# yahoojapan/srgd

Hardware: AMD Instinct MI355X
Metric: HR tiles/sec (256->1024 x4, 50 steps, CFG=1.0) (higher is better)
Workload: dtype bf16; 1 GPU; BASELINE configs[1]: one 256x256 LR tile x4 SR per step, 50 DDPM steps, class_cond_scale=1.0, dim-128 U-Net, bf16, device Philox noise; 5 steps (HR tiles) advance in lock-step so their U-Net tiles share launches; images_in_lockstep=5, step_lanes=1, tiles_per_unet_launch=125, parallelism=image-sharded x1

## Files before the change

### srgd_amd/csrc/conv1x1_bf16.hip

```cpp
#include "conv1x1_epilogue.hpp"

namespace srgd {
namespace {

constexpr int BM1 = 256, BN1 = 128, KC1 = 32, NT1 = 512;
constexpr int A1_BYTES = BM1 * KC1 * 2;
constexpr int B1_BYTES = BN1 * KC1 * 2;
constexpr int STAGE1 = A1_BYTES + B1_BYTES;
constexpr int RING1 = 3;
constexpr int LDS1_BYTES = RING1 * STAGE1;
static_assert(LDS1_BYTES >= EPI_LDS_BYTES && BM1 == EPI_BM && BN1 == EPI_BN && NT1 == EPI_NT, "conv1x1_epilogue.hpp tile shape");

typedef __attribute__((address_space(3))) void* lds_ptr1;
__device__ __forceinline__ void dma16_1(__amdgpu_buffer_rsrc_t rsrc, char* lds_wave_base, int voffset, int soffset) {
  __builtin_amdgcn_raw_ptr_buffer_load_lds(rsrc, (lds_ptr1)lds_wave_base, 16, voffset, soffset, 0, 0);
}
#define WAIT_VM1(N) asm volatile("s_waitcnt vmcnt(" #N ")" ::: "memory")
#define BARRIER1()                       \
  do {                                   \
    __builtin_amdgcn_s_barrier();        \
    __builtin_amdgcn_sched_barrier(0);   \
  } while (0)

struct Conv1Args {
  const bf16* in0; const bf16* in1; int C0, C1;
  int B, Hin, Win;
  int Hout, Wout;
  int KH, KW, stride;
  int ps0, ps1;
  const bf16* w;
  const float* bias;
  int Cout;
  bf16* out;
  const bf16* aux;
  const float* gn_a; const float* gn_b;
  unsigned char* oq; unsigned char* os;
  float* eps4; const float* fin_w; const float* fin_b;
};

__device__ __forceinline__ int row_swz1(int row) { return (row >> 1) & 3; }

template <int EPI>
__global__ __launch_bounds__(NT1, 4) void conv1x1_bf16_kernel(Conv1Args p) {
  extern __shared__ __attribute__((aligned(16))) char smem[];
  const int tid = threadIdx.x;
  const int lane = tid & 63;
  const int wave = __builtin_amdgcn_readfirstlane(tid >> 6);
  const int wm = wave >> 1, wn = wave & 1;
  const int r16 = lane & 15, q16 = lane >> 4;

  const int n_tiles = p.Cout / BN1;
  const int HWo = p.Hout * p.Wout;
  int wg = blockIdx.x;
  {
    const int nwg = gridDim.x, q = nwg >> 3, rem = nwg & 7, x = wg & 7, k = wg >> 3;
    wg = (x < rem ? x * (q + 1) : rem * (q + 1) + (x - rem) * q) + k;
  }
  const int nt = wg % n_tiles;
  const int mt = wg / n_tiles;
  const long m0 = (long)mt * BM1;
  const int b = (int)(m0 / HWo);
  const int p0 = (int)(m0 - (long)b * HWo);
  const int Cin = p.C0 + p.C1;
  const int CC = Cin / KC1;
  const int S = p.KH * p.KW * CC;

#define K_A1_DECL(J)                                                      \
  int a_b0##J, a_b1##J;                                                      \
  {                                                                          \
    const int g = (wave + 8 * J) * 64 + lane;                                \
    const int P = g >> 2;                                                    \
    const int op = p0 + P;                                                   \
    const int oy = op / p.Wout, ox = op - oy * p.Wout;                       \
    const int pix = oy * p.stride * p.Win + ox * p.stride;                   \
    const int sub = (g & 3) ^ row_swz1(P);                                   \
    a_b0##J = (pix * p.ps0 + sub * 8) * 2;                                   \
    a_b1##J = (pix * p.ps1 + sub * 8) * 2;                                   \
  }
  K_A1_DECL(0) K_A1_DECL(1)
#undef K_A1_DECL
  const size_t img0 = (size_t)p.Hin * p.Win * p.ps0, img1 = (size_t)p.Hin * p.Win * p.ps1;
  const __amdgpu_buffer_rsrc_t rs0 =
      __builtin_amdgcn_make_buffer_rsrc((void*)(p.in0 + (size_t)b * img0), 0, (int)(img0 * 2), 0x00020000);
  const __amdgpu_buffer_rsrc_t rs1 = __builtin_amdgcn_make_buffer_rsrc(
      (void*)(p.in1 ? p.in1 + (size_t)b * img1 : p.in0), 0, p.in1 ? (int)(img1 * 2) : 0, 0x00020000);
  const size_t w_tile_stride = (size_t)n_tiles * B1_BYTES;
  const __amdgpu_buffer_rsrc_t rsw = __builtin_amdgcn_make_buffer_rsrc(
      (void*)((const char*)p.w + (size_t)nt * B1_BYTES), 0, (int)((size_t)(S - 1) * w_tile_stride + B1_BYTES), 0x00020000);

  int i_ty = 0, i_tx = 0, i_cc = 0, i_slot = 0, i_w = 0;
  const int tid16 = tid * 16;
  auto issue = [&]() __attribute__((always_inline)) {
    const int c = i_cc * KC1;
    const bool first = c < p.C0;
    const int soff = first ? ((i_ty * p.Win + i_tx) * p.ps0 + c) * 2 : ((i_ty * p.Win + i_tx) * p.ps1 + c - p.C0) * 2;
    char* st = smem + i_slot * STAGE1;
    const int vo0 = first ? a_b00 : a_b10, vo1 = first ? a_b01 : a_b11;
    if (first) {
      dma16_1(rs0, st + wave * 1024, vo0, soff);
      dma16_1(rs0, st + (wave + 8) * 1024, vo1, soff);
    } else {
      dma16_1(rs1, st + wave * 1024, vo0, soff);
      dma16_1(rs1, st + (wave + 8) * 1024, vo1, soff);
    }
    dma16_1(rsw, st + A1_BYTES + wave * 1024, tid16, i_w);
    i_w += (int)w_tile_stride;
    i_slot = i_slot == RING1 - 1 ? 0 : i_slot + 1;
    if (++i_cc == CC) {
      i_cc = 0;
      if (++i_tx == p.KW) { i_tx = 0; ++i_ty; }
    }
  };

  f32x4 c00 = 0, c01 = 0, c02 = 0, c03 = 0, c10 = 0, c11 = 0, c12 = 0, c13 = 0,
        c20 = 0, c21 = 0, c22 = 0, c23 = 0, c30 = 0, c31 = 0, c32 = 0, c33 = 0;
  auto a_addr = [&](int i) {
    const int P = wm * 64 + i * 16 + r16;
    return P * 64 + ((q16 ^ row_swz1(P)) << 4);
  };
  auto b_addr = [&](int j) {
    const int n = wn * 64 + j * 16 + r16;
    return A1_BYTES + n * 64 + ((q16 ^ row_swz1(n)) << 4);
  };
  const int aa0 = a_addr(0), aa1 = a_addr(1), aa2 = a_addr(2), aa3 = a_addr(3);
  const int ba0 = b_addr(0), ba1 = b_addr(1), ba2 = b_addr(2), ba3 = b_addr(3);
  int c_slot = 0;
  auto compute = [&]() __attribute__((always_inline)) {
    const char* st = smem + c_slot * STAGE1;
    c_slot = c_slot == RING1 - 1 ? 0 : c_slot + 1;
    const bf16x8 a0 = *reinterpret_cast<const bf16x8*>(st + aa0);
    const bf16x8 a1 = *reinterpret_cast<const bf16x8*>(st + aa1);
    const bf16x8 a2 = *reinterpret_cast<const bf16x8*>(st + aa2);
    const bf16x8 a3 = *reinterpret_cast<const bf16x8*>(st + aa3);
    const bf16x8 b0 = *reinterpret_cast<const bf16x8*>(st + ba0);
    const bf16x8 b1 = *reinterpret_cast<const bf16x8*>(st + ba1);
    const bf16x8 b2 = *reinterpret_cast<const bf16x8*>(st + ba2);
    const bf16x8 b3 = *reinterpret_cast<const bf16x8*>(st + ba3);
#define MM(C_, A_, B_) C_ = __builtin_amdgcn_mfma_f32_16x16x32_bf16(A_, B_, C_, 0, 0, 0)
    MM(c00, a0, b0); MM(c01, a0, b1); MM(c02, a0, b2); MM(c03, a0, b3);
    MM(c10, a1, b0); MM(c11, a1, b1); MM(c12, a1, b2); MM(c13, a1, b3);
    MM(c20, a2, b0); MM(c21, a2, b1); MM(c22, a2, b2); MM(c23, a2, b3);
    MM(c30, a3, b0); MM(c31, a3, b1); MM(c32, a3, b2); MM(c33, a3, b3);
#undef MM
  };

  issue();
  if (S > 1) issue();
  if (S > 1) WAIT_VM1(3); else WAIT_VM1(0);
  BARRIER1();
  for (int s = 0; s < S; ++s) {
    if (s + 2 < S) issue();
    compute();
    if (s + 2 < S) WAIT_VM1(3); else WAIT_VM1(0);
    BARRIER1();
  }

  conv1x1_epilogue<EPI, BM1>(p, smem, tid, nt, m0, b, p0, c00, c01, c02, c03, c10, c11, c12, c13, c20, c21, c22, c23, c30, c31, c32, c33);
}

}

bool conv1x1_bf16_eligible(const ConvArgs& a) {
  if (a.pad != 0 || a.stride < 1 || a.KH < 1 || a.KW < 1) return false;
  if ((a.Hout - 1) * a.stride + a.KH > a.Hin || (a.Wout - 1) * a.stride + a.KW > a.Win) return false;
  if (a.ps0 % 8 || (a.C1 && (a.ps1 % 8 || a.ps1 < a.C1))) return false;
  if (a.ps0 != a.C0 && (a.C1 || (long)(a.Win - (a.Wout - 1) * a.stride - a.KW) * a.ps0 + a.ps0 < a.C0)) return false;
  if (a.C1 && (a.KH != 1 || a.KW != 1)) return false;
  if (a.C0 % KC1 || a.C1 % KC1 || a.Cout % BN1 || a.Cout != a.CoutPad) return false;
  if (((long)a.Hout * a.Wout) % BM1) return false;
  if (a.gn_partial) return false;
  if (a.mode == CONV_PIXEL_SHUFFLE_SILU && ((a.Cout / 4) % BN1 || a.residual || a.gn_res_src)) return false;
  if (a.mode != CONV_PLAIN && a.mode != CONV_PIXEL_SHUFFLE_SILU) return false;
  if (a.residual && a.gn_res_src) return false;
  if (a.eps4 && (!a.gn_res_src || a.Cout != BN1 || !a.fin_w || !a.fin_b || a.out_q)) return false;
  if ((size_t)a.Hin * a.Win * (size_t)std::max(a.ps0, a.ps1) * 2 >= (1ull << 31)) return false;
  if ((size_t)a.KH * a.KW * ((a.C0 + a.C1) / KC1) * (a.Cout / BN1) * B1_BYTES >= (1ull << 31)) return false;
  return true;
}

void pack_conv1x1_bf16(const float* src_tap_o_i, int taps, int Cin, int Cout, std::vector<unsigned short>& out,
                       unsigned short (*to_bf16)(float)) {
  const int CC = Cin / KC1, NTL = Cout / BN1;
  out.assign((size_t)taps * CC * NTL * BN1 * KC1, 0);
  for (int tap = 0; tap < taps; ++tap)
    for (int cc = 0; cc < CC; ++cc)
      for (int nt = 0; nt < NTL; ++nt) {
        unsigned short* tile = out.data() + ((size_t)(tap * CC + cc) * NTL + nt) * BN1 * KC1;
        for (int n = 0; n < BN1; ++n)
          for (int c = 0; c < 4; ++c) {
            const int cs = c ^ ((n >> 1) & 3);
            for (int e = 0; e < 8; ++e) {
              const int ci = cc * KC1 + c * 8 + e, o = nt * BN1 + n;
              tile[n * KC1 + cs * 8 + e] = to_bf16(src_tap_o_i[((size_t)tap * Cout + o) * Cin + ci]);
            }
          }
      }
}

int conv1x1_bf16(const ConvArgs& a, const void* packed_w, hipStream_t st) {
  if (!conv1x1_bf16_eligible(a)) SRGD_FAIL("conv1x1_bf16: shape not eligible");
  Conv1Args p;
  p.in0 = (const bf16*)a.in0; p.in1 = (const bf16*)a.in1; p.C0 = a.C0; p.C1 = a.C1;
  p.B = a.B; p.Hin = a.Hin; p.Win = a.Win; p.Hout = a.Hout; p.Wout = a.Wout;
  p.KH = a.KH; p.KW = a.KW; p.stride = a.stride; p.ps0 = a.ps0; p.ps1 = a.C1 ? a.ps1 : 0;
  p.w = (const bf16*)packed_w; p.bias = a.bias; p.Cout = a.Cout; p.out = (bf16*)a.out;
  p.aux = a.gn_res_src ? (const bf16*)a.gn_res_src : (const bf16*)a.residual;
  p.gn_a = a.gn_res_a; p.gn_b = a.gn_res_b;
  p.oq = (unsigned char*)a.out_q; p.os = (unsigned char*)a.out_s;
  p.eps4 = a.eps4; p.fin_w = a.fin_w; p.fin_b = a.fin_b;
  if ((p.oq != nullptr) != (p.os != nullptr)) SRGD_FAIL("conv1x1_bf16: MX-fp8 twin needs both the element and the scale buffer");
  const long m_tiles = (long)a.B * a.Hout * a.Wout / BM1;
  const long grid = m_tiles * (a.Cout / BN1);
  if (grid <= 0 || grid > 0x7fffffffL) SRGD_FAIL("conv1x1_bf16: bad grid");
  static bool attr_set[64] = {};
  if (DeviceSetup once(attr_set); once.need) {
#define K_SET1(E_)                                                                                   \
  SRGD_HIP(hipFuncSetAttribute(reinterpret_cast<const void*>(&conv1x1_bf16_kernel<E_>),                 \
                               hipFuncAttributeMaxDynamicSharedMemorySize, LDS1_BYTES));
    K_SET1(EPI_PLAIN) K_SET1(EPI_RESIDUAL) K_SET1(EPI_GNTAIL) K_SET1(EPI_PS_SILU) K_SET1(EPI_GNTAIL_FINAL)
#undef K_SET1
    once.done();
  }
#define K_GO1(E_) hipLaunchKernelGGL((conv1x1_bf16_kernel<E_>), dim3((unsigned)grid), dim3(NT1), LDS1_BYTES, st, p)
  if (a.mode == CONV_PIXEL_SHUFFLE_SILU) K_GO1(EPI_PS_SILU);
  else if (a.gn_res_src && a.eps4) K_GO1(EPI_GNTAIL_FINAL);
  else if (a.gn_res_src) K_GO1(EPI_GNTAIL);
  else if (a.residual) K_GO1(EPI_RESIDUAL);
  else K_GO1(EPI_PLAIN);
#undef K_GO1
  SRGD_HIP(hipGetLastError());
  return 0;
}

}
```

### srgd_amd/csrc/conv1x1_epilogue.hpp

```cpp
#pragma once
#include "kernels.hpp"

namespace srgd {
namespace {

enum { EPI_PLAIN = 0, EPI_RESIDUAL = 1, EPI_GNTAIL = 2, EPI_PS_SILU = 3, EPI_GNTAIL_FINAL = 4 };
constexpr int EPI_BM = 256, EPI_BN = 128, EPI_NT = 512;
constexpr int EPI_ROW = EPI_BN * 2 + 16;
constexpr int EPI_LDS_BYTES = EPI_BM * EPI_ROW;

template <int EPI, int BM, class Args>
__device__ __forceinline__ void conv1x1_epilogue(const Args& p, char* smem, const int tid, const int nt, const long m0, const int b,
                                                 const int p0, const f32x4& c00, const f32x4& c01, const f32x4& c02, const f32x4& c03,
                                                 const f32x4& c10, const f32x4& c11, const f32x4& c12, const f32x4& c13,
                                                 const f32x4& c20, const f32x4& c21, const f32x4& c22, const f32x4& c23,
                                                 const f32x4& c30, const f32x4& c31, const f32x4& c32, const f32x4& c33) {
  constexpr int BM1 = BM, BN1 = EPI_BN, NT1 = BM * 2, EROW1 = EPI_ROW;
  static_assert(BM == 256 || BM == 128, "conv1x1_epilogue: tile of 256 or 128 pixels");
  const int lane = tid & 63;
  const int wave = tid >> 6;
  const int wm = wave >> 1, wn = wave & 1;
  const int r16 = lane & 15, q16 = lane >> 4;
#pragma unroll
  for (int ni = 0; ni < 4; ++ni) {
    const int cl = wn * 64 + ni * 16 + r16;
    const float bias = p.bias ? p.bias[nt * BN1 + cl] : 0.f;
#pragma unroll
    for (int mi = 0; mi < 4; ++mi) {
      const f32x4 av = mi == 0 ? (ni == 0 ? c00 : ni == 1 ? c01 : ni == 2 ? c02 : c03)
                     : mi == 1 ? (ni == 0 ? c10 : ni == 1 ? c11 : ni == 2 ? c12 : c13)
                     : mi == 2 ? (ni == 0 ? c20 : ni == 1 ? c21 : ni == 2 ? c22 : c23)
                               : (ni == 0 ? c30 : ni == 1 ? c31 : ni == 2 ? c32 : c33);
      char* trow = smem + (wm * 64 + mi * 16 + q16 * 4) * EROW1 + cl * 2;
      float v0 = av[0] + bias, v1 = av[1] + bias, v2 = av[2] + bias, v3 = av[3] + bias;
      if (EPI == EPI_PS_SILU) { v0 = silu<false>(v0); v1 = silu<false>(v1); v2 = silu<false>(v2); v3 = silu<false>(v3); }
      typedef __bf16 bf16x2_t __attribute__((ext_vector_type(2)));
      const unsigned own01 = __builtin_bit_cast(unsigned, __builtin_convertvector(f32x2{v0, v1}, bf16x2_t));
      const unsigned own23 = __builtin_bit_cast(unsigned, __builtin_convertvector(f32x2{v2, v3}, bf16x2_t));
      const bool odd_lane = (r16 & 1) != 0;
      const unsigned recv = (unsigned)__builtin_amdgcn_update_dpp(0, (int)(odd_lane ? own01 : own23), 0xB1, 0xf, 0xf, true);
      const unsigned lo_ch = odd_lane ? recv : own01, hi_ch = odd_lane ? own23 : recv;
      char* prow = trow + (odd_lane ? 2 * EROW1 - 2 : 0);
      *reinterpret_cast<unsigned*>(prow) = __builtin_amdgcn_perm(hi_ch, lo_ch, 0x05040100u);
      *reinterpret_cast<unsigned*>(prow + EROW1) = __builtin_amdgcn_perm(hi_ch, lo_ch, 0x07060302u);
    }
  }
  __syncthreads();
  const int col0 = nt * BN1;
  size_t obase;
  int CoutPS = 0, ps_ij = 0, ps_c0 = 0;
  if (EPI == EPI_PS_SILU) {
    CoutPS = p.Cout >> 2;
    ps_ij = col0 / CoutPS;
    ps_c0 = col0 - ps_ij * CoutPS;
  }
  obase = (size_t)m0 * p.Cout + col0;
  float fw0[8], fw1[8], fw2[8];
  if (EPI == EPI_GNTAIL_FINAL) {
#pragma unroll
    for (int e = 0; e < 8; ++e) {
      fw0[e] = p.fin_w[(tid & 15) * 8 + e];
      fw1[e] = p.fin_w[BN1 + (tid & 15) * 8 + e];
      fw2[e] = p.fin_w[2 * BN1 + (tid & 15) * 8 + e];
    }
  }
  constexpr int NCH = (BM1 * 16) / NT1;
  bf16x8 auxv[NCH];
  f32x4 a_lo = {0.f, 0.f, 0.f, 0.f}, a_hi = a_lo, b_lo = a_lo, b_hi = a_lo;
  if (EPI == EPI_RESIDUAL || EPI == EPI_GNTAIL || EPI == EPI_GNTAIL_FINAL) {
#pragma unroll
    for (int i = 0; i < NCH; ++i) {
      const int q = tid + NT1 * i;
      const bf16x8* ap = reinterpret_cast<const bf16x8*>(p.aux + obase + (size_t)(q >> 4) * p.Cout + (q & 15) * 8);
      auxv[i] = __builtin_nontemporal_load(ap);
    }
    if (EPI != EPI_RESIDUAL) {
      const float* ga = p.gn_a + (size_t)b * p.Cout + col0 + (tid & 15) * 8;
      const float* gb = p.gn_b + (size_t)b * p.Cout + col0 + (tid & 15) * 8;
      a_lo = *reinterpret_cast<const f32x4*>(ga); a_hi = *reinterpret_cast<const f32x4*>(ga + 4);
      b_lo = *reinterpret_cast<const f32x4*>(gb); b_hi = *reinterpret_cast<const f32x4*>(gb + 4);
    }
  }
#pragma unroll
  for (int i = 0; i < NCH; ++i) {
    const int q = tid + NT1 * i;
    const int pix = q >> 4, c16 = q & 15;
    bf16x8 v = *reinterpret_cast<const bf16x8*>(smem + pix * EROW1 + c16 * 16);
    if (EPI == EPI_PS_SILU) {
      const int op = p0 + pix;
      const int oy = op / p.Wout, ox = op - oy * p.Wout;
      const size_t o = ((size_t)(b * 2 * p.Hout + 2 * oy + (ps_ij >> 1)) * (2 * p.Wout) + 2 * ox + (ps_ij & 1)) * CoutPS +
                       ps_c0 + c16 * 8;
      __builtin_nontemporal_store(v, reinterpret_cast<bf16x8*>(p.out + o));
      if (p.oq) mx_store_twin(v, p.oq, p.os, o, tid & 3);
    } else {
      const size_t o = obase + (size_t)pix * p.Cout + c16 * 8;
      if (EPI == EPI_RESIDUAL) {
        const bf16x8 rr = auxv[i];
#pragma unroll
        for (int e = 0; e < 8; ++e) v[e] = (bf16)((float)v[e] + (float)rr[e]);
      } else if (EPI == EPI_GNTAIL || EPI == EPI_GNTAIL_FINAL) {
        const bf16x8 hh = auxv[i];
#pragma unroll
        for (int e = 0; e < 8; ++e) {
          const float ca = e < 4 ? a_lo[e & 3] : a_hi[e & 3], cb = e < 4 ? b_lo[e & 3] : b_hi[e & 3];
          v[e] = (bf16)(silu<false>(ca * (float)hh[e] + cb) + (float)v[e]);
        }
      }
      if (EPI == EPI_GNTAIL_FINAL) {
        float s0 = 0.f, s1 = 0.f, s2 = 0.f;
#pragma unroll
        for (int e = 0; e < 8; ++e) {
          const float xv = (float)v[e];
          s0 += xv * fw0[e];
          s1 += xv * fw1[e];
          s2 += xv * fw2[e];
        }
        s0 = row16_sum(s0);
        s1 = row16_sum(s1);
        s2 = row16_sum(s2);
        if (c16 == 0)
          *reinterpret_cast<f32x4*>(p.eps4 + ((size_t)m0 + pix) * 4) = f32x4{s0 + p.fin_b[0], s1 + p.fin_b[1], s2 + p.fin_b[2], 0.f};
        continue;
      }
      __builtin_nontemporal_store(v, reinterpret_cast<bf16x8*>(p.out + o));
      if (p.oq) mx_store_twin(v, p.oq, p.os, o, tid & 3);
    }
  }
}

}
}
```

Before: 1.379 HR tiles/s.

## Make conv1x1 kernel persistent with cross-tile prefetch and round-based epilogue

The 1x1 conv GEMM kernel becomes persistent. The grid is capped at twice the CU count and each workgroup loops over output tiles. The next tile's DMA loads are issued while the current tile's last K-steps compute, which hides the pipeline fill and launch cost per tile. The epilogue is split into four rounds that stage 64 rows at a time through one ring slot instead of the whole LDS, and GN coefficients and final weights are cached in LDS. This adds loop and address bookkeeping plus more registers per thread, which risks occupancy and adds complexity.

Result: no change. 1.382 HR tiles/s, median of 4 (+0.2%).

```diff
diff --git a/srgd_amd/csrc/conv1x1_bf16.hip b/srgd_amd/csrc/conv1x1_bf16.hip
--- a/srgd_amd/csrc/conv1x1_bf16.hip
+++ b/srgd_amd/csrc/conv1x1_bf16.hip
@@ -9,7 +9,7 @@
 constexpr int STAGE1 = A1_BYTES + B1_BYTES;
 constexpr int RING1 = 3;
 constexpr int LDS1_BYTES = RING1 * STAGE1;
-static_assert(LDS1_BYTES >= EPI_LDS_BYTES && BM1 == EPI_BM && BN1 == EPI_BN && NT1 == EPI_NT, "conv1x1_epilogue.hpp tile shape");
+static_assert(STAGE1 >= EPI_RND_LDS && BM1 == EPI_BM && BN1 == EPI_BN && NT1 == EPI_NT, "conv1x1_epilogue.hpp tile shape");
 
 typedef __attribute__((address_space(3))) void* lds_ptr1;
 __device__ __forceinline__ void dma16_1(__amdgpu_buffer_rsrc_t rsrc, char* lds_wave_base, int voffset, int soffset) {
@@ -36,6 +36,7 @@
   const float* gn_a; const float* gn_b;
   unsigned char* oq; unsigned char* os;
   float* eps4; const float* fin_w; const float* fin_b;
+  int n_wg_tiles;
 };
 
 __device__ __forceinline__ int row_swz1(int row) { return (row >> 1) & 3; }
@@ -49,53 +50,61 @@
   const int wm = wave >> 1, wn = wave & 1;
   const int r16 = lane & 15, q16 = lane >> 4;
 
-  const int n_tiles = p.Cout / BN1;
-  const int HWo = p.Hout * p.Wout;
-  int wg = blockIdx.x;
-  {
-    const int nwg = gridDim.x, q = nwg >> 3, rem = nwg & 7, x = wg & 7, k = wg >> 3;
-    wg = (x < rem ? x * (q + 1) : rem * (q + 1) + (x - rem) * q) + k;
-  }
-  const int nt = wg % n_tiles;
-  const int mt = wg / n_tiles;
-  const long m0 = (long)mt * BM1;
-  const int b = (int)(m0 / HWo);
-  const int p0 = (int)(m0 - (long)b * HWo);
+  const unsigned n_tiles = p.Cout / BN1;
+  const unsigned tpi = (unsigned)(p.Hout * p.Wout) / BM1;
   const int Cin = p.C0 + p.C1;
   const int CC = Cin / KC1;
   const int S = p.KH * p.KW * CC;
-
-#define K_A1_DECL(J)                                                      \
-  int a_b0##J, a_b1##J;                                                      \
+  const int T = p.n_wg_tiles;
+  auto tile_of = [&](int v, int& nt_, int& mt_, int& b_, int& p0_) __attribute__((always_inline)) {
+    const int q = T >> 3, rem = T & 7, x = v & 7, k = v >> 3;
+    const unsigned wg = (x < rem ? x * (q + 1) : rem * (q + 1) + (x - rem) * q) + k;
+    nt_ = (int)(wg % n_tiles);
+    mt_ = (int)(wg / n_tiles);
+    b_ = (int)((unsigned)mt_ / tpi);
+    p0_ = (mt_ - b_ * (int)tpi) * BM1;
+  };
+
+  const int a_sub16 = ((lane & 3) ^ ((lane >> 3) & 3)) * 16;
+  int a_px0, a_px1, n_px0 = 0, n_px1 = 0;
+  auto lane_offsets = [&](const int v, int& px0, int& px1) __attribute__((always_inline)) {
+    int nt_, mt_, b_, p0_;
+    tile_of(v < T ? v : 0, nt_, mt_, b_, p0_);
+#define K_A1_SET(J)                                                       \
   {                                                                          \
-    const int g = (wave + 8 * J) * 64 + lane;                                \
-    const int P = g >> 2;                                                    \
-    const int op = p0 + P;                                                   \
+    const int op = p0_ + (((wave + 8 * J) * 64 + lane) >> 2);                \
     const int oy = op / p.Wout, ox = op - oy * p.Wout;                       \
-    const int pix = oy * p.stride * p.Win + ox * p.stride;                   \
-    const int sub = (g & 3) ^ row_swz1(P);                                   \
-    a_b0##J = (pix * p.ps0 + sub * 8) * 2;                                   \
-    a_b1##J = (pix * p.ps1 + sub * 8) * 2;                                   \
-  }
-  K_A1_DECL(0) K_A1_DECL(1)
-#undef K_A1_DECL
-  const size_t img0 = (size_t)p.Hin * p.Win * p.ps0, img1 = (size_t)p.Hin * p.Win * p.ps1;
-  const __amdgpu_buffer_rsrc_t rs0 =
-      __builtin_amdgcn_make_buffer_rsrc((void*)(p.in0 + (size_t)b * img0), 0, (int)(img0 * 2), 0x00020000);
-  const __amdgpu_buffer_rsrc_t rs1 = __builtin_amdgcn_make_buffer_rsrc(
-      (void*)(p.in1 ? p.in1 + (size_t)b * img1 : p.in0), 0, p.in1 ? (int)(img1 * 2) : 0, 0x00020000);
-  const size_t w_tile_stride = (size_t)n_tiles * B1_BYTES;
-  const __amdgpu_buffer_rsrc_t rsw = __builtin_amdgcn_make_buffer_rsrc(
-      (void*)((const char*)p.w + (size_t)nt * B1_BYTES), 0, (int)((size_t)(S - 1) * w_tile_stride + B1_BYTES), 0x00020000);
-
-  int i_ty = 0, i_tx = 0, i_cc = 0, i_slot = 0, i_w = 0;
-  const int tid16 = tid * 16;
-  auto issue = [&]() __attribute__((always_inline)) {
+    px##J = (oy * p.stride * p.Win + ox * p.stride) * 2;                     \
+  }
+    K_A1_SET(0) K_A1_SET(1)
+#undef K_A1_SET
+  };
+  lane_offsets(blockIdx.x, a_px0, a_px1);
+  const int img0 = p.Hin * p.Win * p.ps0, img1 = p.Hin * p.Win * p.ps1;
+  const int w_tile_stride = (int)n_tiles * B1_BYTES;
+
+  int i_v = blockIdx.x, i_ty = 0, i_tx = 0, i_cc = 0, i_slot = 0, i_w = 0;
+  __amdgpu_buffer_rsrc_t rs0, rs1, rsw;
+  auto issue_tile = [&]() __attribute__((always_inline)) {
+    int nt_, mt_, b_, p0_;
+    tile_of(i_v < T ? i_v : 0, nt_, mt_, b_, p0_);
+    rs0 = __builtin_amdgcn_make_buffer_rsrc((void*)(p.in0 + (size_t)b_ * img0), 0, img0 * 2, 0x00020000);
+    rs1 = __builtin_amdgcn_make_buffer_rsrc((void*)(p.in1 ? p.in1 + (size_t)b_ * img1 : p.in0), 0, p.in1 ? img1 * 2 : 0, 0x00020000);
+    rsw = __builtin_amdgcn_make_buffer_rsrc((void*)((const char*)p.w + (size_t)nt_ * B1_BYTES), 0,
+                                            (S - 1) * w_tile_stride + B1_BYTES, 0x00020000);
+    i_ty = i_tx = i_cc = 0;
+    i_w = 0;
+  };
+  issue_tile();
+  const int lane16 = lane * 16;
+  auto issue = [&]() __attribute__((always_inline)) -> bool {
+    if (i_v >= T) return false;
     const int c = i_cc * KC1;
     const bool first = c < p.C0;
     const int soff = first ? ((i_ty * p.Win + i_tx) * p.ps0 + c) * 2 : ((i_ty * p.Win + i_tx) * p.ps1 + c - p.C0) * 2;
     char* st = smem + i_slot * STAGE1;
-    const int vo0 = first ? a_b00 : a_b10, vo1 = first ? a_b01 : a_b11;
+    const int ps = first ? p.ps0 : p.ps1;
+    const int vo0 = a_px0 * ps + a_sub16, vo1 = a_px1 * ps + a_sub16;
     if (first) {
       dma16_1(rs0, st + wave * 1024, vo0, soff);
       dma16_1(rs0, st + (wave + 8) * 1024, vo1, soff);
@@ -103,39 +112,38 @@
       dma16_1(rs1, st + wave * 1024, vo0, soff);
       dma16_1(rs1, st + (wave + 8) * 1024, vo1, soff);
     }
-    dma16_1(rsw, st + A1_BYTES + wave * 1024, tid16, i_w);
-    i_w += (int)w_tile_stride;
+    dma16_1(rsw, st + A1_BYTES + wave * 1024, lane16, i_w + wave * 1024);
+    i_w += w_tile_stride;
     i_slot = i_slot == RING1 - 1 ? 0 : i_slot + 1;
     if (++i_cc == CC) {
       i_cc = 0;
-      if (++i_tx == p.KW) { i_tx = 0; ++i_ty; }
+      if (++i_tx == p.KW) {
+        i_tx = 0;
+        if (++i_ty == p.KH) {
+          i_v += gridDim.x;
+          a_px0 = n_px0; a_px1 = n_px1;
+          issue_tile();
+        }
+      }
     }
-  };
-
-  f32x4 c00 = 0, c01 = 0, c02 = 0, c03 = 0, c10 = 0, c11 = 0, c12 = 0, c13 = 0,
-        c20 = 0, c21 = 0, c22 = 0, c23 = 0, c30 = 0, c31 = 0, c32 = 0, c33 = 0;
-  auto a_addr = [&](int i) {
-    const int P = wm * 64 + i * 16 + r16;
-    return P * 64 + ((q16 ^ row_swz1(P)) << 4);
-  };
-  auto b_addr = [&](int j) {
-    const int n = wn * 64 + j * 16 + r16;
-    return A1_BYTES + n * 64 + ((q16 ^ row_swz1(n)) << 4);
-  };
-  const int aa0 = a_addr(0), aa1 = a_addr(1), aa2 = a_addr(2), aa3 = a_addr(3);
-  const int ba0 = b_addr(0), ba1 = b_addr(1), ba2 = b_addr(2), ba3 = b_addr(3);
+    return true;
+  };
+
+  f32x4 c00, c01, c02, c03, c10, c11, c12, c13, c20, c21, c22, c23, c30, c31, c32, c33;
+  const int aa0 = (wm * 64 + r16) * 64 + ((q16 ^ row_swz1(r16)) << 4);
+  const int ba0 = A1_BYTES + (wn * 64 + r16) * 64 + ((q16 ^ row_swz1(r16)) << 4);
   int c_slot = 0;
   auto compute = [&]() __attribute__((always_inline)) {
     const char* st = smem + c_slot * STAGE1;
     c_slot = c_slot == RING1 - 1 ? 0 : c_slot + 1;
     const bf16x8 a0 = *reinterpret_cast<const bf16x8*>(st + aa0);
-    const bf16x8 a1 = *reinterpret_cast<const bf16x8*>(st + aa1);
-    const bf16x8 a2 = *reinterpret_cast<const bf16x8*>(st + aa2);
-    const bf16x8 a3 = *reinterpret_cast<const bf16x8*>(st + aa3);
+    const bf16x8 a1 = *reinterpret_cast<const bf16x8*>(st + aa0 + 1024);
+    const bf16x8 a2 = *reinterpret_cast<const bf16x8*>(st + aa0 + 2048);
+    const bf16x8 a3 = *reinterpret_cast<const bf16x8*>(st + aa0 + 3072);
     const bf16x8 b0 = *reinterpret_cast<const bf16x8*>(st + ba0);
-    const bf16x8 b1 = *reinterpret_cast<const bf16x8*>(st + ba1);
-    const bf16x8 b2 = *reinterpret_cast<const bf16x8*>(st + ba2);
-    const bf16x8 b3 = *reinterpret_cast<const bf16x8*>(st + ba3);
+    const bf16x8 b1 = *reinterpret_cast<const bf16x8*>(st + ba0 + 1024);
+    const bf16x8 b2 = *reinterpret_cast<const bf16x8*>(st + ba0 + 2048);
+    const bf16x8 b3 = *reinterpret_cast<const bf16x8*>(st + ba0 + 3072);
 #define MM(C_, A_, B_) C_ = __builtin_amdgcn_mfma_f32_16x16x32_bf16(A_, B_, C_, 0, 0, 0)
     MM(c00, a0, b0); MM(c01, a0, b1); MM(c02, a0, b2); MM(c03, a0, b3);
     MM(c10, a1, b0); MM(c11, a1, b1); MM(c12, a1, b2); MM(c13, a1, b3);
@@ -144,18 +152,31 @@
 #undef MM
   };
 
-  issue();
-  if (S > 1) issue();
-  if (S > 1) WAIT_VM1(3); else WAIT_VM1(0);
+  bool more = issue();
+  more = issue() && more;
+  if (more) WAIT_VM1(3); else WAIT_VM1(0);
   BARRIER1();
-  for (int s = 0; s < S; ++s) {
-    if (s + 2 < S) issue();
-    compute();
-    if (s + 2 < S) WAIT_VM1(3); else WAIT_VM1(0);
-    BARRIER1();
-  }
-
-  conv1x1_epilogue<EPI, BM1>(p, smem, tid, nt, m0, b, p0, c00, c01, c02, c03, c10, c11, c12, c13, c20, c21, c22, c23, c30, c31, c32, c33);
+  for (int v = blockIdx.x; v < T; v += gridDim.x) {
+    int nt, mt, b, p0;
+    tile_of(v, nt, mt, b, p0);
+    lane_offsets(v + (int)gridDim.x, n_px0, n_px1);
+    c00 = 0; c01 = 0; c02 = 0; c03 = 0; c10 = 0; c11 = 0; c12 = 0; c13 = 0;
+    c20 = 0; c21 = 0; c22 = 0; c23 = 0; c30 = 0; c31 = 0; c32 = 0; c33 = 0;
+    for (int s = 0; s < S; ++s) {
+      const bool issued = issue();
+      compute();
+      if (s == 0 && v != (int)blockIdx.x) { if (issued) WAIT_VM1(11); else WAIT_VM1(8); }
+      else if (issued) WAIT_VM1(3);
+      else WAIT_VM1(0);
+      BARRIER1();
+    }
+    char* stg = smem + (c_slot == 0 ? RING1 - 1 : c_slot - 1) * STAGE1;
+    int tid_e = tid;
+    asm volatile("" : "+v"(tid_e));
+    conv1x1_epilogue_rounds<EPI>(p, stg, tid_e, nt, (long)mt * BM1, b, p0, c00, c01, c02, c03, c10, c11, c12, c13, c20, c21, c22, c23,
+                                 c30, c31, c32, c33);
+    EPI_LDS_BARRIER();
+  }
 }
 
 }
@@ -167,6 +188,7 @@
   if (a.ps0 != a.C0 && (a.C1 || (long)(a.Win - (a.Wout - 1) * a.stride - a.KW) * a.ps0 + a.ps0 < a.C0)) return false;
   if (a.C1 && (a.KH != 1 || a.KW != 1)) return false;
   if (a.C0 % KC1 || a.C1 % KC1 || a.Cout % BN1 || a.Cout != a.CoutPad) return false;
+  if (a.KH * a.KW * ((a.C0 + a.C1) / KC1) < 2) return false;
   if (((long)a.Hout * a.Wout) % BM1) return false;
   if (a.gn_partial) return false;
   if (a.mode == CONV_PIXEL_SHUFFLE_SILU && ((a.Cout / 4) % BN1 || a.residual || a.gn_res_src)) return false;
@@ -210,8 +232,19 @@
   p.eps4 = a.eps4; p.fin_w = a.fin_w; p.fin_b = a.fin_b;
   if ((p.oq != nullptr) != (p.os != nullptr)) SRGD_FAIL("conv1x1_bf16: MX-fp8 twin needs both the element and the scale buffer");
   const long m_tiles = (long)a.B * a.Hout * a.Wout / BM1;
-  const long grid = m_tiles * (a.Cout / BN1);
-  if (grid <= 0 || grid > 0x7fffffffL) SRGD_FAIL("conv1x1_bf16: bad grid");
+  const long tiles = m_tiles * (a.Cout / BN1);
+  if (tiles <= 0 || tiles > 0x7fff0000L) SRGD_FAIL("conv1x1_bf16: bad grid");
+  p.n_wg_tiles = (int)tiles;
+  static int cus[64] = {};
+  int dev = 0;
+  SRGD_HIP(hipGetDevice(&dev));
+  if (dev >= 0 && dev < 64 && cus[dev] == 0) {
+    int n = 0;
+    SRGD_HIP(hipDeviceGetAttribute(&n, hipDeviceAttributeMultiprocessorCount, dev));
+    __atomic_store_n(&cus[dev], n > 8 ? n & ~7 : 8, __ATOMIC_RELAXED);
+  }
+  const int slots = 2 * ((dev >= 0 && dev < 64) ? cus[dev] : 256);
+  const long grid = tiles <= slots ? tiles : slots;
   static bool attr_set[64] = {};
   if (DeviceSetup once(attr_set); once.need) {
 #define K_SET1(E_)                                                                                   \
diff --git a/srgd_amd/csrc/conv1x1_epilogue.hpp b/srgd_amd/csrc/conv1x1_epilogue.hpp
--- a/srgd_amd/csrc/conv1x1_epilogue.hpp
+++ b/srgd_amd/csrc/conv1x1_epilogue.hpp
@@ -8,6 +8,67 @@
 constexpr int EPI_BM = 256, EPI_BN = 128, EPI_NT = 512;
 constexpr int EPI_ROW = EPI_BN * 2 + 16;
 constexpr int EPI_LDS_BYTES = EPI_BM * EPI_ROW;
+constexpr int EPI_RND_BYTES = 64 * EPI_ROW;
+constexpr int EPI_RND_LDS = EPI_RND_BYTES + 5 * EPI_BN * 4;
+
+#define EPI_LDS_BARRIER() asm volatile("s_waitcnt lgkmcnt(0)\n\ts_barrier" ::: "memory")
+
+template <int EPI>
+__device__ __forceinline__ void epi_pack_block(const f32x4 av, const float bias, const int r16, unsigned& w0, unsigned& w1) {
+  float v0 = av[0] + bias, v1 = av[1] + bias, v2 = av[2] + bias, v3 = av[3] + bias;
+  if (EPI == EPI_PS_SILU) { v0 = silu<false>(v0); v1 = silu<false>(v1); v2 = silu<false>(v2); v3 = silu<false>(v3); }
+  typedef __bf16 bf16x2_t __attribute__((ext_vector_type(2)));
+  const unsigned own01 = __builtin_bit_cast(unsigned, __builtin_convertvector(f32x2{v0, v1}, bf16x2_t));
+  const unsigned own23 = __builtin_bit_cast(unsigned, __builtin_convertvector(f32x2{v2, v3}, bf16x2_t));
+  const bool odd_lane = (r16 & 1) != 0;
+  const unsigned recv = (unsigned)__builtin_amdgcn_update_dpp(0, (int)(odd_lane ? own01 : own23), 0xB1, 0xf, 0xf, true);
+  const unsigned lo_ch = odd_lane ? recv : own01, hi_ch = odd_lane ? own23 : recv;
+  w0 = __builtin_amdgcn_perm(hi_ch, lo_ch, 0x05040100u);
+  w1 = __builtin_amdgcn_perm(hi_ch, lo_ch, 0x07060302u);
+}
+__device__ __forceinline__ void epi_write_block(const unsigned w0, const unsigned w1, char* trow, const int r16) {
+  char* prow = trow + ((r16 & 1) ? 2 * EPI_ROW - 2 : 0);
+  *reinterpret_cast<unsigned*>(prow) = w0;
+  *reinterpret_cast<unsigned*>(prow + EPI_ROW) = w1;
+}
+template <int EPI>
+__device__ __forceinline__ void epi_stage_block(const f32x4 av, const float bias, char* trow, const int r16) {
+  unsigned w0, w1;
+  epi_pack_block<EPI>(av, bias, r16, w0, w1);
+  epi_write_block(w0, w1, trow, r16);
+}
+
+template <int EPI, int FWS, class Args>
+__device__ __forceinline__ void epi_chunk_store(const Args& p, bf16x8 v, const bf16x8 tail, const f32x4 a_lo, const f32x4 a_hi,
+                                                const f32x4 b_lo, const f32x4 b_hi, const float* fw, const size_t o,
+                                                const size_t gpix, const int c16, const int tid) {
+  if (EPI == EPI_RESIDUAL) {
+#pragma unroll
+    for (int e = 0; e < 8; ++e) v[e] = (bf16)((float)v[e] + (float)tail[e]);
+  } else if (EPI == EPI_GNTAIL || EPI == EPI_GNTAIL_FINAL) {
+#pragma unroll
+    for (int e = 0; e < 8; ++e) {
+      const float ca = e < 4 ? a_lo[e & 3] : a_hi[e & 3], cb = e < 4 ? b_lo[e & 3] : b_hi[e & 3];
+      v[e] = (bf16)(silu<false>(ca * (float)tail[e] + cb) + (float)v[e]);
+    }
+  }
+  if (EPI == EPI_GNTAIL_FINAL) {
+    float s0 = 0.f, s1 = 0.f, s2 = 0.f;
+#pragma unroll
+    for (int e = 0; e < 8; ++e) s0 += (float)v[e] * fw[e];
+#pragma unroll
+    for (int e = 0; e < 8; ++e) s1 += (float)v[e] * fw[FWS + e];
+#pragma unroll
+    for (int e = 0; e < 8; ++e) s2 += (float)v[e] * fw[2 * FWS + e];
+    s0 = row16_sum(s0);
+    s1 = row16_sum(s1);
+    s2 = row16_sum(s2);
+    if (c16 == 0) *reinterpret_cast<f32x4*>(p.eps4 + gpix * 4) = f32x4{s0 + p.fin_b[0], s1 + p.fin_b[1], s2 + p.fin_b[2], 0.f};
+    return;
+  }
+  __builtin_nontemporal_store(v, reinterpret_cast<bf16x8*>(p.out + o));
+  if (p.oq) mx_store_twin(v, p.oq, p.os, o, tid & 3);
+}
 
 template <int EPI, int BM, class Args>
 __device__ __forceinline__ void conv1x1_epilogue(const Args& p, char* smem, const int tid, const int nt, const long m0, const int b,
@@ -31,41 +92,29 @@
                      : mi == 1 ? (ni == 0 ? c10 : ni == 1 ? c11 : ni == 2 ? c12 : c13)
                      : mi == 2 ? (ni == 0 ? c20 : ni == 1 ? c21 : ni == 2 ? c22 : c23)
                                : (ni == 0 ? c30 : ni == 1 ? c31 : ni == 2 ? c32 : c33);
-      char* trow = smem + (wm * 64 + mi * 16 + q16 * 4) * EROW1 + cl * 2;
-      float v0 = av[0] + bias, v1 = av[1] + bias, v2 = av[2] + bias, v3 = av[3] + bias;
-      if (EPI == EPI_PS_SILU) { v0 = silu<false>(v0); v1 = silu<false>(v1); v2 = silu<false>(v2); v3 = silu<false>(v3); }
-      typedef __bf16 bf16x2_t __attribute__((ext_vector_type(2)));
-      const unsigned own01 = __builtin_bit_cast(unsigned, __builtin_convertvector(f32x2{v0, v1}, bf16x2_t));
-      const unsigned own23 = __builtin_bit_cast(unsigned, __builtin_convertvector(f32x2{v2, v3}, bf16x2_t));
-      const bool odd_lane = (r16 & 1) != 0;
-      const unsigned recv = (unsigned)__builtin_amdgcn_update_dpp(0, (int)(odd_lane ? own01 : own23), 0xB1, 0xf, 0xf, true);
-      const unsigned lo_ch = odd_lane ? recv : own01, hi_ch = odd_lane ? own23 : recv;
-      char* prow = trow + (odd_lane ? 2 * EROW1 - 2 : 0);
-      *reinterpret_cast<unsigned*>(prow) = __builtin_amdgcn_perm(hi_ch, lo_ch, 0x05040100u);
-      *reinterpret_cast<unsigned*>(prow + EROW1) = __builtin_amdgcn_perm(hi_ch, lo_ch, 0x07060302u);
+      epi_stage_block<EPI>(av, bias, smem + (wm * 64 + mi * 16 + q16 * 4) * EROW1 + cl * 2, r16);
     }
   }
   __syncthreads();
   const int col0 = nt * BN1;
-  size_t obase;
   int CoutPS = 0, ps_ij = 0, ps_c0 = 0;
   if (EPI == EPI_PS_SILU) {
     CoutPS = p.Cout >> 2;
     ps_ij = col0 / CoutPS;
     ps_c0 = col0 - ps_ij * CoutPS;
   }
-  obase = (size_t)m0 * p.Cout + col0;
-  float fw0[8], fw1[8], fw2[8];
+  const size_t obase = (size_t)m0 * p.Cout + col0;
+  float fw[24] = {};
   if (EPI == EPI_GNTAIL_FINAL) {
 #pragma unroll
     for (int e = 0; e < 8; ++e) {
-      fw0[e] = p.fin_w[(tid & 15) * 8 + e];
-      fw1[e] = p.fin_w[BN1 + (tid & 15) * 8 + e];
-      fw2[e] = p.fin_w[2 * BN1 + (tid & 15) * 8 + e];
+      fw[e] = p.fin_w[(tid & 15) * 8 + e];
+      fw[8 + e] = p.fin_w[BN1 + (tid & 15) * 8 + e];
+      fw[16 + e] = p.fin_w[2 * BN1 + (tid & 15) * 8 + e];
     }
   }
   constexpr int NCH = (BM1 * 16) / NT1;
-  bf16x8 auxv[NCH];
+  bf16x8 auxv[NCH] = {};
   f32x4 a_lo = {0.f, 0.f, 0.f, 0.f}, a_hi = a_lo, b_lo = a_lo, b_hi = a_lo;
   if (EPI == EPI_RESIDUAL || EPI == EPI_GNTAIL || EPI == EPI_GNTAIL_FINAL) {
 #pragma unroll
@@ -85,49 +134,104 @@
   for (int i = 0; i < NCH; ++i) {
     const int q = tid + NT1 * i;
     const int pix = q >> 4, c16 = q & 15;
-    bf16x8 v = *reinterpret_cast<const bf16x8*>(smem + pix * EROW1 + c16 * 16);
+    const bf16x8 v = *reinterpret_cast<const bf16x8*>(smem + pix * EROW1 + c16 * 16);
+    size_t o = obase + (size_t)pix * p.Cout + c16 * 8;
     if (EPI == EPI_PS_SILU) {
       const int op = p0 + pix;
       const int oy = op / p.Wout, ox = op - oy * p.Wout;
-      const size_t o = ((size_t)(b * 2 * p.Hout + 2 * oy + (ps_ij >> 1)) * (2 * p.Wout) + 2 * ox + (ps_ij & 1)) * CoutPS +
-                       ps_c0 + c16 * 8;
-      __builtin_nontemporal_store(v, reinterpret_cast<bf16x8*>(p.out + o));
-      if (p.oq) mx_store_twin(v, p.oq, p.os, o, tid & 3);
-    } else {
-      const size_t o = obase + (size_t)pix * p.Cout + c16 * 8;
-      if (EPI == EPI_RESIDUAL) {
-        const bf16x8 rr = auxv[i];
-#pragma unroll
-        for (int e = 0; e < 8; ++e) v[e] = (bf16)((float)v[e] + (float)rr[e]);
-      } else if (EPI == EPI_GNTAIL || EPI == EPI_GNTAIL_FINAL) {
-        const bf16x8 hh = auxv[i];
-#pragma unroll
-        for (int e = 0; e < 8; ++e) {
-          const float ca = e < 4 ? a_lo[e & 3] : a_hi[e & 3], cb = e < 4 ? b_lo[e & 3] : b_hi[e & 3];
-          v[e] = (bf16)(silu<false>(ca * (float)hh[e] + cb) + (float)v[e]);
-        }
+      o = ((size_t)(b * 2 * p.Hout + 2 * oy + (ps_ij >> 1)) * (2 * p.Wout) + 2 * ox + (ps_ij & 1)) * CoutPS + ps_c0 + c16 * 8;
+    }
+    epi_chunk_store<EPI, 8>(p, v, auxv[i], a_lo, a_hi, b_lo, b_hi, fw, o, (size_t)m0 + pix, c16, tid);
+  }
+}
+
+template <int EPI, class Args>
+__device__ __forceinline__ void conv1x1_epilogue_rounds(const Args& p, char* stg, const int tid, const int nt, const long m0,
+                                                        const int b, const int p0, const f32x4& c00, const f32x4& c01,
+                                                        const f32x4& c02, const f32x4& c03, const f32x4& c10, const f32x4& c11,
+                                                        const f32x4& c12, const f32x4& c13, const f32x4& c20, const f32x4& c21,
+                                                        const f32x4& c22, const f32x4& c23, const f32x4& c30, const f32x4& c31,
+                                                        const f32x4& c32, const f32x4& c33) {
+  constexpr int BN1 = EPI_BN, EROW1 = EPI_ROW;
+  const int lane = tid & 63;
+  const int wave = tid >> 6;
+  const int wm = wave >> 1, wn = wave & 1;
+  const int r16 = lane & 15, q16 = lane >> 4;
+  const int col0 = nt * BN1;
+  const int c16 = tid & 15, r0 = tid >> 4;
+  int CoutPS = 0, ps_ij = 0, ps_c0 = 0;
+  if (EPI == EPI_PS_SILU) {
+    CoutPS = p.Cout >> 2;
+    ps_ij = col0 / CoutPS;
+    ps_c0 = col0 - ps_ij * CoutPS;
+  }
+  const size_t obase = (size_t)m0 * p.Cout + col0;
+  float bias4[4];
+#pragma unroll
+  for (int ni = 0; ni < 4; ++ni) bias4[ni] = p.bias ? p.bias[col0 + wn * 64 + ni * 16 + r16] : 0.f;
+  unsigned w0[16], w1[16];
+#pragma unroll
+  for (int mi = 0; mi < 4; ++mi) {
+#pragma unroll
+    for (int ni = 0; ni < 4; ++ni) {
+      const f32x4 av = mi == 0 ? (ni == 0 ? c00 : ni == 1 ? c01 : ni == 2 ? c02 : c03)
+                     : mi == 1 ? (ni == 0 ? c10 : ni == 1 ? c11 : ni == 2 ? c12 : c13)
+                     : mi == 2 ? (ni == 0 ? c20 : ni == 1 ? c21 : ni == 2 ? c22 : c23)
+                               : (ni == 0 ? c30 : ni == 1 ? c31 : ni == 2 ? c32 : c33);
+      epi_pack_block<EPI>(av, bias4[ni], r16, w0[mi * 4 + ni], w1[mi * 4 + ni]);
+    }
+  }
+  bf16x8 auxv[8] = {};
+  auto load_tail = [&](const int k) __attribute__((always_inline)) {
+    const int R = r0 + 32 * (k & 1), pix = (R >> 4) * 64 + (k >> 1) * 16 + (R & 15);
+    auxv[k] = __builtin_nontemporal_load(reinterpret_cast<const bf16x8*>(p.aux + obase + (size_t)pix * p.Cout + c16 * 8));
+  };
+  constexpr bool TAIL = EPI == EPI_RESIDUAL || EPI == EPI_GNTAIL || EPI == EPI_GNTAIL_FINAL;
+  if (TAIL) {
+#pragma unroll
+    for (int k = 0; k < 2; ++k) load_tail(k);
+  }
+  float* coef_lds = reinterpret_cast<float*>(stg + EPI_RND_BYTES);
+  float* fin_lds = coef_lds + 2 * BN1;
+  if ((EPI == EPI_GNTAIL || EPI == EPI_GNTAIL_FINAL) && tid < 2 * BN1)
+    coef_lds[tid] = (tid < BN1 ? p.gn_a : p.gn_b)[(size_t)b * p.Cout + col0 + (tid & (BN1 - 1))];
+  if (EPI == EPI_GNTAIL_FINAL && tid < 3 * BN1) fin_lds[tid] = p.fin_w[tid];
+#pragma unroll
+  for (int mi = 0; mi < 4; ++mi) {
+    if (mi) EPI_LDS_BARRIER();
+#pragma unroll
+    for (int ni = 0; ni < 4; ++ni)
+      epi_write_block(w0[mi * 4 + ni], w1[mi * 4 + ni], stg + (wm * 16 + q16 * 4) * EROW1 + (wn * 64 + ni * 16 + r16) * 2, r16);
+    EPI_LDS_BARRIER();
+    constexpr bool TAIL_LATE = EPI == EPI_GNTAIL_FINAL;
+    if (TAIL && !TAIL_LATE && mi < 3) {
+      load_tail(2 * mi + 2);
+      load_tail(2 * mi + 3);
+    }
+#pragma unroll
+    for (int i = 0; i < 2; ++i) {
+      const int R = r0 + 32 * i, pix = (R >> 4) * 64 + mi * 16 + (R & 15);
+      const bf16x8 v = *reinterpret_cast<const bf16x8*>(stg + R * EROW1 + c16 * 16);
+      f32x4 a_lo = {0.f, 0.f, 0.f, 0.f}, a_hi = a_lo, b_lo = a_lo, b_hi = a_lo;
+      if (EPI == EPI_GNTAIL || EPI == EPI_GNTAIL_FINAL) {
+        a_lo = *reinterpret_cast<const f32x4*>(coef_lds + c16 * 8); a_hi = *reinterpret_cast<const f32x4*>(coef_lds + c16 * 8 + 4);
+        b_lo = *reinterpret_cast<const f32x4*>(coef_lds + BN1 + c16 * 8); b_hi = *reinterpret_cast<const f32x4*>(coef_lds + BN1 + c16 * 8 + 4);
       }
-      if (EPI == EPI_GNTAIL_FINAL) {
-        float s0 = 0.f, s1 = 0.f, s2 = 0.f;
-#pragma unroll
-        for (int e = 0; e < 8; ++e) {
-          const float xv = (float)v[e];
-          s0 += xv * fw0[e];
-          s1 += xv * fw1[e];
-          s2 += xv * fw2[e];
-        }
-        s0 = row16_sum(s0);
-        s1 = row16_sum(s1);
-        s2 = row16_sum(s2);
-        if (c16 == 0)
-          *reinterpret_cast<f32x4*>(p.eps4 + ((size_t)m0 + pix) * 4) = f32x4{s0 + p.fin_b[0], s1 + p.fin_b[1], s2 + p.fin_b[2], 0.f};
-        continue;
+      size_t o = obase + (size_t)pix * p.Cout + c16 * 8;
+      if (EPI == EPI_PS_SILU) {
+        const int op = p0 + pix;
+        const int oy = op / p.Wout, ox = op - oy * p.Wout;
+        o = ((size_t)(b * 2 * p.Hout + 2 * oy + (ps_ij >> 1)) * (2 * p.Wout) + 2 * ox + (ps_ij & 1)) * CoutPS + ps_c0 + c16 * 8;
       }
-      __builtin_nontemporal_store(v, reinterpret_cast<bf16x8*>(p.out + o));
-      if (p.oq) mx_store_twin(v, p.oq, p.os, o, tid & 3);
-    }
-  }
-}
-
-}
-}
+      epi_chunk_store<EPI, BN1>(p, v, auxv[mi * 2 + i], a_lo, a_hi, b_lo, b_hi, fin_lds + c16 * 8, o, (size_t)m0 + pix, c16, tid);
+    }
+    if (TAIL && TAIL_LATE && mi < 3) {
+      asm volatile("" ::: "memory");
+      load_tail(2 * mi + 2);
+      load_tail(2 * mi + 3);
+    }
+  }
+}
+
+}
+}
```
